# isaac-sim/IsaacGymEnvs

Measured on AMD Instinct MI355X. Metric: env-steps/sec (num_envs x control-steps/sec), random-action rollout, higher is better.
Workload: dtype f32; 1 GPU; Ant num_envs=4096 per GPU (4096 total), VecTask.step() via Python API, actions = 2*torch.rand-1 drawn before every step (README.md:48-51), seed 42+rank; 11000 untimed settle steps (about 0.5 s of back-to-back stepping at the BASELINE size) precede the 5 warm-ups; task=Ant, num_envs_per_gpu=4096, parallelism=env-shard x1, multi_wave=16, fused_sub=1, fused_post=1

## Files before the change

### isaacgymenvs_amd/csrc/core/engine_mw.hpp

```cpp
#pragma once
#include "engine.hpp"

namespace mi {

template <class M>
struct SimMW : Sim<M> {
    using B = Sim<M>;
    using typename B::Ctx;
    using typename B::BodyTmp;
    static constexpr int NB = B::NB, ND = B::ND, NV = B::NV, OFF = B::OFF, NSPH = B::NSPH, NSENS = B::NSENS, NLIM = B::NLIM,
                         NROWG = B::NROWG, NVA = B::NVA, NR = M::NROLE;

    static constexpr int role_of_body(int b) { return M::role_of_limb[M::limb_of_body[b]]; }
    static constexpr int role_of_gi(int gi) { return gi < OFF ? -1 : role_of_body(M::dof_body[gi - OFF]); }
    static constexpr bool trunk_body(int b) { return role_of_body(b) < 0; }
    static constexpr bool trunk_gi(int gi) { return role_of_gi(gi) < 0; }
    template <int R> static constexpr bool owns_body(int b) { return role_of_body(b) == R || (trunk_body(b) && R == M::TRUNK_ROLE); }
    template <int R> static constexpr bool owns_gi(int gi) { return role_of_gi(gi) == R || (trunk_gi(gi) && R == M::TRUNK_ROLE); }
    template <int R> static constexpr bool sees_gi(int gi) { return role_of_gi(gi) == R || trunk_gi(gi); }
    static constexpr int NTB = []() constexpr { int n = 0; for (int b = 0; b < NB; ++b) n += trunk_body(b) ? 1 : 0; return n; }();
    static constexpr int tslot(int b) { int n = 0; for (int k = 0; k < b; ++k) n += trunk_body(k) ? 1 : 0; return n; }
    static constexpr int NVT = []() constexpr { int n = 0; for (int i = 0; i < NV; ++i) n += trunk_gi(i) ? 1 : 0; return n; }();
    static constexpr int tidx(int gi) { int n = 0; for (int k = 0; k < gi; ++k) n += trunk_gi(k) ? 1 : 0; return n; }
    static constexpr int entry_row(int e) {
        for (int i = 0; i < NV; ++i)
            for (int j = 0; j <= i; ++j)
                if (M::midx[i][j] == e) return i;
        return 0;
    }
    static constexpr bool trunk_entry(int e) { return trunk_gi(entry_row(e)); }
    static constexpr int NTE = []() constexpr { int n = 0; for (int e = 0; e < M::NM; ++e) n += trunk_entry(e) ? 1 : 0; return n; }();
    static constexpr int teidx(int e) { int n = 0; for (int k = 0; k < e; ++k) n += trunk_entry(k) ? 1 : 0; return n; }
    static constexpr bool limb_root(int b) { return b > 0 && !trunk_body(b) && trunk_body(M::parent[b]); }
    static constexpr int NLR = []() constexpr { int n = 0; for (int b = 0; b < NB; ++b) n += limb_root(b) ? 1 : 0; return n; }();
    static constexpr int lridx(int b) { int n = 0; for (int k = 0; k < b; ++k) n += limb_root(k) ? 1 : 0; return n; }
    static constexpr int X_LR = B::ROW_SLOTS_STATIC;
    static constexpr int X_DT = X_LR + 16 * NLR;
    static constexpr int X_DY = X_DT + NR * NTE;
    static constexpr int X_DW = X_DY + NR * NVT;
    static constexpr int X_FLG = X_DW + 2 * NR * NVT;
    static constexpr int X_AT = X_FLG + 2 * NR;
    static constexpr int MW_SLOTS = X_AT + NROWG;

    static constexpr int NUNIT = NLIM + NSPH;
    template <int R> static constexpr bool own_unit(int u) {
        if (u < 0 || u >= NUNIT) return false;
        return u < NLIM ? owns_gi<R>(OFF + B::limdof(u)) : owns_body<R>(M::sph_body[u - NLIM]);
    }
    template <int R> static constexpr int next_own(int u) {
        for (int k = u + 1; k < NUNIT; ++k) if (own_unit<R>(k)) return k;
        return NUNIT;
    }
    template <int R> static constexpr int own_pos(int u) { int n = 0; for (int k = 0; k < u; ++k) n += own_unit<R>(k) ? 1 : 0; return n; }

    template <int R, int b, int XLR, int RS>
    MI_HD void trunk_down(const SimParams& P, Ctx& c, BodyTmp (&tb)[NTB], const float* Rp, const float* rp, const float* Vp,
                          const float* Ap, const RowStore<RS> rows) {
        constexpr int ts = tslot(b);
        BodyTmp& t = tb[ts];
        this->template body_down<b>(P, c, Rp, rp, Vp, Ap, t);
        sfor<NB>([&](auto C_) MI_LAMBDA {
            constexpr int ch = C_;
            if constexpr (ch > b) if constexpr (M::parent[ch] == b) {
                if constexpr (trunk_body(ch)) {
                    trunk_down<R, ch, XLR>(P, c, tb, t.Rb, t.rb, t.Vc, t.Ac, rows);
                } else if constexpr (role_of_body(ch) == R) {
                    SpI Ic;
                    float Fc[6];
                    this->template body_pass<ch>(P, c, t.Rb, t.rb, t.Vc, t.Ac, Ic, Fc);
                    constexpr int o = XLR + 16 * lridx(ch);
                    rows(o) = Ic.m;
                    sfor<3>([&](auto K) MI_LAMBDA { rows(o + 1 + K) = Ic.h[K]; });
                    sfor<6>([&](auto K) MI_LAMBDA { rows(o + 4 + K) = Ic.I[K]; rows(o + 10 + K) = Fc[K]; });
                }
            }
        });
    }

    template <int R, bool KEEP = false, int RS, class GND, class BAR>
    MI_HD void substep_role(const SimParams& P, const float* tau, const float h, const RowStore<RS> rows, const Strided lamc,
                            const Strided laml, const Strided sensor, const Strided dof_force, const GND& gnd, const float mu_env,
                            const Strided netf, const int stage, const BAR& bar) {
        static_assert(!M::FIXED, "multi-wave sub-step: free-base models");
        auto G = [&](int row, int cc) MI_LAMBDA -> float& { return rows(row * M::MAXCHAIN + cc); };
        auto Ainv = [&](int row) MI_LAMBDA -> float& { return rows(NROWG * M::MAXCHAIN + row); };
        auto vt = [&](int row) MI_LAMBDA -> float& { return rows(NROWG * M::MAXCHAIN + NROWG + row); };
        auto lam = [&](int row) MI_LAMBDA -> float& { return rows(NROWG * M::MAXCHAIN + 2 * NROWG + row); };
        const float invh = MI_RCP(h);
        float (&root)[13] = this->root;
        float (&q)[M::NDA] = this->q;
        float (&qd)[M::NDA] = this->qd;
#if defined(MI_TIMING)
        unsigned long long* const tstamp = this->tstamp;
#endif
        MI_STAMP(0);
        Ctx c;
        float (&S)[M::NDA][6] = c.S;
        float (&L)[M::NM] = c.L;
        if (stage == 0) {
            sfor<ND>([&](auto D) MI_LAMBDA {
                constexpr int d = D;
                if constexpr (M::dof_limited[d] && owns_gi<R>(OFF + d)) { constexpr int o = B::stage_slot_lim(d); rows(o) = laml(d); }
            });
            sfor<3 * NSPH>([&](auto K) MI_LAMBDA {
                if constexpr (owns_body<R>(M::sph_body[K / 3])) { constexpr int o = B::stage_slot_con(K); rows(o) = lamc(K); }
            });
        }
        BodyTmp tb[NTB];
        static_assert(!B::COMPACT && B::LAM_IN_ROWS, "substep_role: models on the static row store");
        trunk_down<R, 0, X_LR>(P, c, tb, nullptr, nullptr, nullptr, nullptr, rows);
        MI_PHASE();
        float Ldi[NVA], y[NVA], w[NVA], v[NVA];
        v[0] = root[7]; v[1] = root[8]; v[2] = root[9]; v[3] = root[10]; v[4] = root[11]; v[5] = root[12];
        sfor<ND>([&](auto D) MI_LAMBDA { v[OFF + D] = qd[D]; });
        sfor<M::NM>([&](auto E_) MI_LAMBDA { if constexpr (trunk_entry(E_)) L[E_] = 0.f; });
        sfor<NV>([&](auto I) MI_LAMBDA { if constexpr (trunk_gi(I)) y[I] = 0.f; });
        float sc_damp[M::NDA], sc_stiff[M::NDA], sc_arm[M::NDA];
        sfor<ND>([&](auto D) MI_LAMBDA { sc_damp[D] = 1.f; sc_stiff[D] = 1.f; sc_arm[D] = 1.f; });
        if constexpr (B::SCALED) {
            if (this->actor_scale.p != nullptr) {
                sfor<ND>([&](auto D) MI_LAMBDA {
                    if constexpr (sees_gi<R>(OFF + D)) {
                        sc_damp[D] = this->actor_scale(B::AS_DAMP + D); sc_stiff[D] = this->actor_scale(B::AS_STIFF + D); sc_arm[D] = this->actor_scale(B::AS_ARM + D);
                    }
                });
            }
        }
        sfor<ND>([&](auto D) MI_LAMBDA {
            constexpr int d = D, gi = OFF + d;
            if constexpr (role_of_gi(gi) == R) {
                const float K = M::dof_stiffness[d] * sc_stiff[d], Dm = M::dof_damping[d] * sc_damp[d];
                L[M::midx[gi][gi]] += M::dof_armature[d] * sc_arm[d] + h * Dm + h * h * K;
                y[gi] = tau[d] - c.bias[gi] - K * (q[d] - M::dof_springref[d]) - (Dm + h * K) * qd[d];
            }
        });
        auto factor = [&](auto K_) MI_LAMBDA {
            constexpr int k = decltype(K_)::value;
            const float dk2 = fmaxf(L[M::midx[k][k]], 1e-30f);
            const float inv = MI_RSQ(dk2);
            L[M::midx[k][k]] = dk2 * inv;
            Ldi[k] = inv;
            sfor<M::nanc[k]>([&](auto A_) MI_LAMBDA { L[M::midx[k][M::anc[k][A_]]] *= inv; });
            sfor<M::nanc[k]>([&](auto A_) MI_LAMBDA {
                constexpr int i = M::anc[k][A_];
                const float lki = L[M::midx[k][i]];
                L[M::midx[i][i]] -= lki * lki;
                sfor<M::nanc[i]>([&](auto B_) MI_LAMBDA {
                    constexpr int j = M::anc[i][B_];
                    L[M::midx[i][j]] -= lki * L[M::midx[k][j]];
                });
            });
        };
        auto whiten = [&](auto I_) MI_LAMBDA {
            constexpr int i = decltype(I_)::value;
            const float z = y[i] * Ldi[i];
            sfor<M::nanc[i]>([&](auto A_) MI_LAMBDA { y[M::anc[i][A_]] -= L[M::midx[i][M::anc[i][A_]]] * z; });
            float s = L[M::midx[i][i]] * v[i];
            sfor<M::nanc[i]>([&](auto A_) MI_LAMBDA { s += L[M::midx[i][M::anc[i][A_]]] * v[M::anc[i][A_]]; });
            w[i] = s + h * z;
        };
        sfor_rev<NV>([&](auto K_) MI_LAMBDA { if constexpr (role_of_gi(K_) == R) factor(K_); });
        MI_PHASE();
        sfor_rev<NV>([&](auto I_) MI_LAMBDA { if constexpr (role_of_gi(I_) == R) whiten(I_); });
        sfor<M::NM>([&](auto E_) MI_LAMBDA { if constexpr (trunk_entry(E_)) { constexpr int o = X_DT + R * NTE + teidx(E_); rows(o) = L[E_]; } });
        sfor<NV>([&](auto I) MI_LAMBDA { if constexpr (trunk_gi(I)) { constexpr int o = X_DY + R * NVT + tidx(I); rows(o) = y[I]; } });
// ... 86 lines not shown
                        g[kk] -= L[M::midx[i][j]] * z;
                    });
                });
                float al = P.cfm, at = 0.f;
                sfor<M::nanc[gi] + 1>([&](auto K) MI_LAMBDA {
                    constexpr int k = K, i = (k == 0) ? gi : M::anc[gi][k == 0 ? 0 : k - 1];
                    if constexpr (trunk_gi(i)) at += g[k] * g[k]; else al += g[k] * g[k];
                    G(row, k) = g[k];
                });
                Ainv(row) = al;
                rows(X_AT + row) = at;
                const float vtl = (C >= 0.f) ? -C * invh : fminf(-C * P.erp * invh, P.max_depen_vel);
                vt(row) = vtl;
                lam(row) = l0;
                act = ((l0 > 0.f) || (vtl > 0.f)) ? 1.f : act;
                wadd(std::integral_constant<int, gi>{}, g[0] * l0);
                sfor<M::nanc[gi]>([&](auto A_) MI_LAMBDA { wadd(std::integral_constant<int, M::anc[gi][A_]>{}, g[1 + A_] * l0); });
            }
        });
        MI_PHASE();
        unsigned long long sph_active = 0ull;
        sfor<NSPH>([&](auto S_) MI_LAMBDA {
            constexpr int s = S_, b = M::sph_body[s], row0 = NLIM + 3 * s;
            if constexpr (owns_body<R>(b)) {
                MI_PHASE();
                const float* cs = c.xcs[s];
                float xc[3], dist;
                float fr[3][3];
                if constexpr (GND::HEIGHTFIELD) {
                    gnd.contact(root[0] + cs[0], root[1] + cs[1], root[2] + cs[2], M::sph_rad[s], &dist, fr[0]);
                    contact_frame(fr[0], fr[1], fr[2]);
                    sfor<3>([&](auto K) MI_LAMBDA { xc[K] = cs[K] - M::sph_rad[s] * fr[0][K]; });
                } else {
                    xc[0] = cs[0]; xc[1] = cs[1]; xc[2] = cs[2] - M::sph_rad[s];
                    dist = (root[2] + xc[2]) - P.ground_z;
                }
                const bool on = dist < P.contact_offset;
                const float onf = on ? 1.f : 0.f;
                const float gap = dist - P.rest_offset;
                if (!MI_WAVE_ANY(on)) {
                    sfor<3>([&](auto K) MI_LAMBDA { lam(row0 + K) = 0.f; });
                    return;
                }
                sph_active |= 1ull << s;
                act = on ? 1.f : act;
                sfor<3>([&](auto K) MI_LAMBDA {
                    constexpr int k = K, row = row0 + k;
                    float W[6];
                    if constexpr (GND::HEIGHTFIELD) {
                        cross3(xc, fr[k], W);
                        W[3] = fr[k][0]; W[4] = fr[k][1]; W[5] = fr[k][2];
                    } else {
                        constexpr int ax = (k == 0) ? 2 : (k == 1 ? 0 : 1);
                        sfor<6>([&](auto I_) MI_LAMBDA { W[I_] = 0.f; });
                        W[3 + ax] = 1.f;
                        if constexpr (ax == 0) { W[1] = xc[2]; W[2] = -xc[1]; }
                        else if constexpr (ax == 1) { W[0] = -xc[2]; W[2] = xc[0]; }
                        else { W[0] = xc[1]; W[1] = -xc[0]; }
                    }
                    float g[M::MAXCHAIN];
                    sfor<M::chain_len[b]>([&](auto C) MI_LAMBDA {
                        constexpr int gi = M::chain[b][C];
                        if constexpr (gi >= OFF) g[C] = dot6(S[gi - OFF], W);
                        else if constexpr (gi < 3) g[C] = W[3 + gi];
                        else g[C] = W[gi - 3];
                    });
                    chain_solve(std::integral_constant<int, b>{}, g);
                    float al = P.cfm, at = 0.f;
                    sfor<M::chain_len[b]>([&](auto C) MI_LAMBDA {
                        if constexpr (trunk_gi(M::chain[b][C])) at += g[C] * g[C]; else al += g[C] * g[C];
                        G(row, C) = g[C];
                    });
                    Ainv(row) = on ? al : __builtin_inff();
                    rows(X_AT + row) = at;
                    const float vtn = (gap >= 0.f) ? -gap * invh : fminf(-gap * P.erp * invh, P.max_depen_vel);
                    if constexpr (GND::HEIGHTFIELD) vt(row) = (k == 0) ? vtn : fr[0][k - 1];
                    else vt(row) = (k == 0) ? vtn : 0.f;
                    const float l0 = lam(row) * P.warm * onf;
                    lam(row) = l0;
                    sfor<M::chain_len[b]>([&](auto C) MI_LAMBDA { wadd(std::integral_constant<int, M::chain[b][C]>{}, g[C] * l0); });
                });
            }
        });
        sfor<NVT>([&](auto I) MI_LAMBDA { rows(X_DW + R * NVT + I) = dw[I]; });
        rows(X_FLG + R) = act;
        MI_STAMP(3);
        bar();
        MI_STAMP(4);
        sfor<NV>([&](auto I) MI_LAMBDA {
            constexpr int i = I;
            if constexpr (trunk_gi(i)) { sfor<NR>([&](auto R_) MI_LAMBDA { constexpr int o = X_DW + R_ * NVT + tidx(i); w[i] += rows(o); }); }
        });
        {
            struct UBuf { float g[3][M::MAXCHAIN]; float al[3], at[3], vt, lam[3]; };
            UBuf ub[2];
            float wtl[NVT];
            for (int it = 0; it < P.iters; ++it) {
                int zero;
                MI_OPAQUE_ZERO(zero);
                const RowStore<RS> rit = rows.shifted(zero);
                const int par = it & 1;
                const RowStore<RS> xout = rows.shifted((X_DW + (par ^ 1) * NR * NVT) * RowStore<RS>::stride);
                const RowStore<RS> fin = rows.shifted((X_FLG + par * NR) * RowStore<RS>::stride), fout = rows.shifted((X_FLG + (par ^ 1) * NR) * RowStore<RS>::stride);
                float nact = 0.f;
                sfor<NR>([&](auto R_) MI_LAMBDA { nact += fin(R_); });
                const float om = (nact > 1.5f) ? 0.5f * (nact + 1.f) : 1.f;
                const float iom = 1.f / om;
                sfor<NV>([&](auto I) MI_LAMBDA { if constexpr (trunk_gi(I)) { constexpr int ti = tidx(I); wtl[ti] = w[I]; } });
                auto wget = [&](auto GI) MI_LAMBDA -> float {
                    constexpr int gi = decltype(GI)::value;
                    if constexpr (trunk_gi(gi)) { constexpr int ti = tidx(gi); return wtl[ti]; } else return w[gi];
                };
                auto wupd = [&](auto GI, const float val) MI_LAMBDA {
                    constexpr int gi = decltype(GI)::value;
                    if constexpr (trunk_gi(gi)) { constexpr int ti = tidx(gi); wtl[ti] += om * val; } else w[gi] += val;
                };
                float actn = 0.f;
                auto load_unit = [&](auto U_, UBuf& Bf) MI_LAMBDA {
                    constexpr int u = decltype(U_)::value;
                    if constexpr (u < NLIM) {
                        constexpr int d = B::limdof(u), gi = OFF + d, row = u;
                        sfor<M::nanc[gi] + 1>([&](auto K) MI_LAMBDA { Bf.g[0][K] = rit(row * M::MAXCHAIN + K); });
                        Bf.al[0] = rit(NROWG * M::MAXCHAIN + row);
                        Bf.at[0] = rit(X_AT + row);
                        Bf.vt = rit(NROWG * M::MAXCHAIN + NROWG + row);
                        Bf.lam[0] = rit(NROWG * M::MAXCHAIN + 2 * NROWG + row);
                    } else if constexpr (u < NUNIT) {
                        constexpr int s = u - NLIM, b = M::sph_body[s], row0 = NLIM + 3 * s;
                        sfor<3>([&](auto K) MI_LAMBDA {
                            sfor<M::chain_len[b]>([&](auto C) MI_LAMBDA { Bf.g[K][C] = rit((row0 + K) * M::MAXCHAIN + C); });
                            Bf.al[K] = rit(NROWG * M::MAXCHAIN + row0 + K);
                            Bf.at[K] = rit(X_AT + row0 + K);
                            Bf.lam[K] = rit(NROWG * M::MAXCHAIN + 2 * NROWG + row0 + K);
                        });
                        Bf.vt = rit(NROWG * M::MAXCHAIN + NROWG + row0);
                    }
                };
                auto unit_on = [&](auto U_) MI_LAMBDA -> bool {
                    constexpr int u = decltype(U_)::value;
                    if constexpr (u < NLIM) return true;
                    else if constexpr (u < NUNIT) return (sph_active >> (u - NLIM) & 1ull) != 0ull;
                    else return false;
                };
                constexpr int U0 = next_own<R>(-1);
                if constexpr (U0 < NUNIT) load_unit(std::integral_constant<int, U0>{}, ub[0]);
                sfor<NUNIT>([&](auto U_) MI_LAMBDA {
                    constexpr int u = U_;
                    if constexpr (own_unit<R>(u)) {
                        constexpr int pos = own_pos<R>(u), un = next_own<R>(u);
                        UBuf& Bf = ub[pos & 1];
                        if (unit_on(std::integral_constant<int, un>{}))
                            load_unit(std::integral_constant<int, un>{}, ub[(pos + 1) & 1]);
                        MI_PHASE();
                        if (!unit_on(std::integral_constant<int, u>{})) return;
                        if constexpr (u < NLIM) {
                            constexpr int d = B::limdof(u), gi = OFF + d, row = u;
                            float vn = Bf.g[0][0] * wget(std::integral_constant<int, gi>{});
                            sfor<M::nanc[gi]>([&](auto A_) MI_LAMBDA { vn += Bf.g[0][1 + A_] * wget(std::integral_constant<int, M::anc[gi][A_]>{}); });
                            const float lo = Bf.lam[0];
                            const float nl = fmaxf(lo - (vn - Bf.vt) * MI_RCP(Bf.al[0] + om * Bf.at[0]), 0.f);
                            const float dl = nl - lo;
                            lam(row) = nl;
                            actn = (nl > 0.f) ? 1.f : actn;
                            wupd(std::integral_constant<int, gi>{}, Bf.g[0][0] * dl);
                            sfor<M::nanc[gi]>([&](auto A_) MI_LAMBDA { wupd(std::integral_constant<int, M::anc[gi][A_]>{}, Bf.g[0][1 + A_] * dl); });
                        } else {
                            constexpr int s = u - NLIM, b = M::sph_body[s], row0 = NLIM + 3 * s;
                            const float mu = 0.5f * ((mu_env >= 0.f ? mu_env : M::sph_mu[s]) + P.plane_mu);
                            float ainv[3];
                            sfor<3>([&](auto K) MI_LAMBDA { ainv[K] = MI_RCP(Bf.al[K] + om * Bf.at[K]); });
                            float ln;
                            {
                                float vn = 0.f;
                                sfor<M::chain_len[b]>([&](auto C) MI_LAMBDA { vn += Bf.g[0][C] * wget(std::integral_constant<int, M::chain[b][C]>{}); });
                                const float lo = Bf.lam[0];
                                ln = fmaxf(lo - (vn - Bf.vt) * ainv[0], 0.f);
                                const float dl = ln - lo;
                                lam(row0) = ln;
                                actn = (ln > 0.f) ? 1.f : actn;
                                sfor<M::chain_len[b]>([&](auto C) MI_LAMBDA { wupd(std::integral_constant<int, M::chain[b][C]>{}, Bf.g[0][C] * dl); });
                            }
                            float lt[2], vtg[2];
                            sfor<2>([&](auto K) MI_LAMBDA {
                                float vn = 0.f;
                                sfor<M::chain_len[b]>([&](auto C) MI_LAMBDA { vn += Bf.g[1 + K][C] * wget(std::integral_constant<int, M::chain[b][C]>{}); });
                                vtg[K] = vn;
                                lt[K] = Bf.lam[1 + K] - vn * ainv[1 + K];
                            });
                            friction_disc(lt, Bf.lam[1], Bf.lam[2], vtg[0], vtg[1], ainv[1], ainv[2], mu * ln);
                            sfor<2>([&](auto K) MI_LAMBDA {
                                constexpr int row = row0 + 1 + K;
                                const float nl = lt[K], dl = nl - Bf.lam[1 + K];
                                lam(row) = nl;
                                sfor<M::chain_len[b]>([&](auto C) MI_LAMBDA { wupd(std::integral_constant<int, M::chain[b][C]>{}, Bf.g[1 + K][C] * dl); });
                            });
                        }
                    }
                });
                sfor<NV>([&](auto I) MI_LAMBDA { if constexpr (trunk_gi(I)) { constexpr int ti = tidx(I); xout(R * NVT + ti) = (wtl[ti] - w[I]) * iom; } });
                fout(R) = actn;
                bar();
                sfor<NV>([&](auto I) MI_LAMBDA {
                    constexpr int i = I;
                    if constexpr (trunk_gi(i)) { sfor<NR>([&](auto R_) MI_LAMBDA { constexpr int o = R_ * NVT + tidx(i); w[i] += xout(o); }); }
                });
            }
        }
        MI_STAMP(5);
        sfor<NV>([&](auto I_) MI_LAMBDA {
            constexpr int i = I_;
            if constexpr (sees_gi<R>(i)) {
                float s = w[i];
                sfor<M::nanc[i]>([&](auto A_) MI_LAMBDA { s -= L[M::midx[i][M::anc[i][A_]]] * v[M::anc[i][A_]]; });
                v[i] = s * Ldi[i];
            }
        });
        MI_PHASE();
        sfor<ND>([&](auto D) MI_LAMBDA {
            constexpr int d = D;
            if constexpr (owns_gi<R>(OFF + d)) {
                float ll = 0.f;
                if constexpr (M::dof_limited[d]) {
                    constexpr int row = B::limrow(d);
                    const float dl = q[d] - this->template limit_lower<d>(), du = this->template limit_upper<d>() - q[d];
                    ll = (dl < du) ? lam(row) : -lam(row);
                    if constexpr (KEEP) lam(row) = ll;
                }
                laml(d) = ll;
                dof_force(d) = tau[d] - M::dof_stiffness[d] * sc_stiff[d] * (q[d] - M::dof_springref[d]) - M::dof_damping[d] * sc_damp[d] * v[OFF + d] + ll * invh;
            }
        });
        float sens[6 * M::NSENSA];
        sfor<6 * NSENS>([&](auto K) MI_LAMBDA { sens[K] = 0.f; });
        float nf[GND::NETF ? NB : 1][3];
        if constexpr (GND::NETF) sfor<NB>([&](auto B_) MI_LAMBDA { nf[B_][0] = nf[B_][1] = nf[B_][2] = 0.f; });
        sfor<NSPH>([&](auto S_) MI_LAMBDA {
            constexpr int s = S_, b = M::sph_body[s], row0 = NLIM + 3 * s;
            if constexpr (owns_body<R>(b)) {
                if (!(sph_active >> s & 1ull)) {
                    lamc(3 * s) = 0.f; lamc(3 * s + 1) = 0.f; lamc(3 * s + 2) = 0.f;
                    return;
                }
                const float ln = lam(row0), l1 = lam(row0 + 1), l2 = lam(row0 + 2);
                lamc(3 * s) = ln; lamc(3 * s + 1) = l1; lamc(3 * s + 2) = l2;
                float f[3], xc[3];
                if constexpr (GND::HEIGHTFIELD) {
                    float n[3], t1[3], t2[3];
                    n[0] = vt(row0 + 1); n[1] = vt(row0 + 2);
                    n[2] = MI_SQRT(fmaxf(1.f - n[0] * n[0] - n[1] * n[1], 0.f));
                    contact_frame(n, t1, t2);
                    sfor<3>([&](auto K) MI_LAMBDA {
                        f[K] = (n[K] * ln + t1[K] * l1 + t2[K] * l2) * invh;
                        xc[K] = c.xcs[s][K] - M::sph_rad[s] * n[K];
                        nf[b][K] += f[K];
                    });
                } else {
                    f[0] = l1 * invh; f[1] = l2 * invh; f[2] = ln * invh;
                    xc[0] = c.xcs[s][0]; xc[1] = c.xcs[s][1]; xc[2] = c.xcs[s][2] - M::sph_rad[s];
                    if constexpr (GND::NETF) sfor<3>([&](auto K) MI_LAMBDA { nf[b][K] += f[K]; });
                }
                if constexpr (B::sensor_of(b) >= 0) {
                    constexpr int k = B::sensor_of(b);
                    const float arm[3] = {xc[0] - c.rs[k][0], xc[1] - c.rs[k][1], xc[2] - c.rs[k][2]};
                    float tq[3], fl[3], tl[3];
                    cross3(arm, f, tq);
                    matTvec3(c.Rs[k], f, fl); matTvec3(c.Rs[k], tq, tl);
                    sfor<3>([&](auto C) MI_LAMBDA { sens[6 * k + C] += fl[C]; sens[6 * k + 3 + C] += tl[C]; });
                }
            }
        });
        if constexpr (GND::NETF) sfor<NB>([&](auto B_) MI_LAMBDA {
            if constexpr (owns_body<R>(B_)) sfor<3>([&](auto K) MI_LAMBDA { netf(3 * B_ + K) = nf[B_][K]; });
        });
        sfor<NSENS>([&](auto K_) MI_LAMBDA {
            if constexpr (owns_body<R>(M::sens_body[K_])) sfor<6>([&](auto C) MI_LAMBDA { sensor(6 * K_ + C) = sens[6 * K_ + C]; });
        });
        MI_PHASE();
        sfor<ND>([&](auto D) MI_LAMBDA {
            if constexpr (owns_gi<R>(OFF + D)) { qd[D] = v[OFF + D]; q[D] += h * qd[D]; }
        });
        if constexpr (R == M::TRUNK_ROLE) {
#if !defined(MI_NO_VEL_CLAMP)
            {
                const float w2 = v[3] * v[3] + v[4] * v[4] + v[5] * v[5], l2 = v[0] * v[0] + v[1] * v[1] + v[2] * v[2];
                const float sw = (w2 > kMaxAngularVelocity * kMaxAngularVelocity) ? kMaxAngularVelocity * MI_RSQ(w2) : 1.f;
                const float sl = (l2 > kMaxLinearVelocity * kMaxLinearVelocity) ? kMaxLinearVelocity * MI_RSQ(l2) : 1.f;
                v[0] *= sl; v[1] *= sl; v[2] *= sl; v[3] *= sw; v[4] *= sw; v[5] *= sw;
            }
#endif
            sfor<3>([&](auto K) MI_LAMBDA { root[7 + K] = v[K]; root[10 + K] = v[3 + K]; root[K] += h * v[K]; });
            const float om[3] = {v[3], v[4], v[5]};
            const float an = MI_SQRT(dot3(om, om)), th = an * h;
            float dq[4];
            {
                float sn, cs;
                sincosf(0.5f * th, &sn, &cs);
                const bool big = th > 1e-12f;
                const float k = big ? sn * MI_RCP(fmaxf(an, 1e-30f)) : 0.5f * h;
                dq[0] = om[0] * k; dq[1] = om[1] * k; dq[2] = om[2] * k; dq[3] = big ? cs : 1.f;
            }
            float* Q = root + 3;
            const float x = dq[3] * Q[0] + dq[0] * Q[3] + dq[1] * Q[2] - dq[2] * Q[1];
            const float yy = dq[3] * Q[1] - dq[0] * Q[2] + dq[1] * Q[3] + dq[2] * Q[0];
            const float z = dq[3] * Q[2] + dq[0] * Q[1] - dq[1] * Q[0] + dq[2] * Q[3];
            const float ww = dq[3] * Q[3] - dq[0] * Q[0] - dq[1] * Q[1] - dq[2] * Q[2];
            const float n = MI_RSQ(x * x + yy * yy + z * z + ww * ww);
            Q[0] = x * n; Q[1] = yy * n; Q[2] = z * n; Q[3] = ww * n;
        }
        MI_STAMP(6);
    }
};

}
```

### isaacgymenvs_amd/csrc/mw_kernels.hpp

```cpp
#pragma once
#include "step_kernels.hpp"
#include "core/engine_mw.hpp"
#include "tasks/anymal_step.hpp"

namespace mi {

#if defined(MI_TIMING)
__device__ unsigned long long* g_mi_tstamp_mw = nullptr;
#endif
struct DevBarrier {
    __device__ __forceinline__ void operator()() const { __syncthreads(); }
};
template <class M, int E>
constexpr size_t mw_lds_bytes() { return (size_t)SimMW<M>::MW_SLOTS * E * sizeof(float); }
template <class M, class GND, int E, int R>
__device__ __forceinline__ void mw_role(const View& v, const SimParams& P, const ActParams& ap, const float* __restrict__ actions_in,
                                        const int src, const GND& gnd, float* lds_rows, const int e, const int lane, float* post_x = nullptr) {
    using S = SimMW<M>;
    constexpr int ND = M::ND;
    const int N = v.N;
    S sim;
    load_sim(sim, v, e);
    load_actor_scales(sim, v, e);
    float tau[M::NDA];
// ... 18 lines not shown
                    t = fminf(fmaxf(u, -ap.torque_limit), ap.torque_limit);
                }
            }
            tau[k] = t;
            if constexpr (mine) v.tau[k * N + e] = t;
        });
    } else {
        sfor<ND>([&](auto K) MI_LAMBDA { tau[K] = v.tau[K * N + e]; });
    }
    {
        typedef const __attribute__((address_space(1))) void* gptr_t;
        typedef __attribute__((address_space(3))) void* lptr_t;
        float* slot0 = lds_rows;
        sfor<ND>([&](auto D) MI_LAMBDA {
            constexpr int d = D;
            if constexpr (M::dof_limited[d] && S::template owns_gi<R>(M::OFF + d)) {
                constexpr int o = Sim<M>::stage_slot_lim(d) * E;
                __builtin_amdgcn_global_load_lds((gptr_t)(v.laml + (size_t)d * N + e), (lptr_t)(slot0 + o), 4, 0, 0);
            }
        });
        sfor<3 * M::NSPH>([&](auto K) MI_LAMBDA {
            if constexpr (S::template owns_body<R>(M::sph_body[K / 3])) {
                constexpr int o = Sim<M>::stage_slot_con(K) * E;
                __builtin_amdgcn_global_load_lds((gptr_t)(v.lamc + (size_t)K * N + e), (lptr_t)(slot0 + o), 4, 0, 0);
            }
        });
    }
    const float h = P.dt / (float)P.substeps;
    const Strided lamc{v.lamc + e, N}, laml{v.laml + e, N}, sensor{v.sensor + e, N}, dof_force{v.dof_force + e, N};
    const Strided netf{GND::NETF ? v.netf + e : nullptr, N};
    const float mu_env = (GND::HEIGHTFIELD || v.friction != nullptr) ? v.friction[e] : -1.f;
    sim.template substep_role<R>(P, tau, h, RowStore<E>{lds_rows + lane}, lamc, laml, sensor, dof_force, gnd, mu_env, netf, true, DevBarrier{});
    sfor<ND>([&](auto K) MI_LAMBDA {
        if constexpr (S::template owns_gi<R>(M::OFF + K)) {
            v.dof[K * N + e] = sim.q[K];
            v.dof[(ND + K) * N + e] = sim.qd[K];
        }
    });
    if constexpr (R == M::TRUNK_ROLE) sfor<13>([&](auto K) MI_LAMBDA { v.root[K * N + e] = sim.root[K]; });
    if (post_x != nullptr) {
        sfor<ND>([&](auto K) MI_LAMBDA {
            if constexpr (S::template owns_gi<R>(M::OFF + K)) { post_x[(13 + K) * E] = sim.q[K]; post_x[(13 + ND + K) * E] = sim.qd[K]; }
        });
        if constexpr (R == M::TRUNK_ROLE) sfor<13>([&](auto K) MI_LAMBDA { post_x[K * E] = sim.root[K]; });
    }
}
template <class M, class GND, int E>
__global__ __launch_bounds__(64 * M::NROLE) void substep_mw_kernel(View v, SimParams P, ActParams ap, const float* __restrict__ actions_in,
                                                                   int src, GND gnd) {
    extern __shared__ float lds_rows[];
    static_assert(M::NROLE == 4, "four roles, one per SIMD of a CU");
    const int lane = threadIdx.x;
    if (lane >= E) return;
    const int e = xcd_env_base<E>(blockIdx.x) + lane;
    if (e >= v.N) return;
    const int role = __builtin_amdgcn_readfirstlane(threadIdx.y);
    switch (role) {
        case 0: mw_role<M, GND, E, 0>(v, P, ap, actions_in, src, gnd, lds_rows, e, lane); break;
        case 1: mw_role<M, GND, E, 1>(v, P, ap, actions_in, src, gnd, lds_rows, e, lane); break;
        case 2: mw_role<M, GND, E, 2>(v, P, ap, actions_in, src, gnd, lds_rows, e, lane); break;
        default: mw_role<M, GND, E, 3>(v, P, ap, actions_in, src, gnd, lds_rows, e, lane); break;
    }
}

template <class GND>
struct MwFusedArgs {
    View v;
    SimParams P;
    ActParams ap;
    const float* actions_in;
    int first, rest, n_sub, tail;
    GND gnd;
    int cmdnorm = 0, cmdnorm_allow_knee = 0;
    float cmdnorm_max_len = 0.f;
};
template <class M, int E>
constexpr size_t mw_fused_lds_bytes() { return (size_t)(SimMW<M>::MW_SLOTS + 13) * E * sizeof(float); }
template <class GND>
struct MwFusedPostArgs {
    MwFusedArgs<GND> f;
    LocoParams tp;
};
template <class S, class M, bool HUM, int E, int R, bool BAR_FIRST = false>
__device__ __forceinline__ void loco_post_role(const View& v, const LocoParams& tp, S& sim, const float* act, const int e, float* xpost) {
    using T = Loco<M::ND, 6 * M::NSENS, HUM>;
    constexpr int ND = M::ND, NOBS = T::NOBS;
    const int N = v.N;
    if constexpr (BAR_FIRST) __syncthreads();
    const uint32_t genv = (uint32_t)(v.env_offset + e);
    const bool do_reset = v.reset[e] != 0;
    int ep = v.episode[e];
    float* ob = v.obs + (size_t)e * NOBS;
    float* oc = v.obs_out + ((size_t)v.ring * N + e) * NOBS;
    const float c = v.clip_obs;
    auto put = [&](const int k, const float x) MI_LAMBDA { ob[k] = x; oc[k] = fminf(fmaxf(x, -c), c); };
    sfor<ND>([&](auto D) MI_LAMBDA {
        constexpr int d = D;
        if constexpr (S::template owns_gi<R>(M::OFF + d)) {
            if (do_reset) {
                T::reset_dof(tp, v.seed, genv, (uint32_t)ep, d, tp.initial_dof_pos[d], tp.dof_lower[d], tp.dof_upper[d], &sim.q[d], &sim.qd[d]);
                v.laml[d * N + e] = 0.f;
            }
            v.dof[d * N + e] = sim.q[d];
            v.dof[(ND + d) * N + e] = sim.qd[d];
            float ps, vs, fs;
            T::obs_dof(tp, sim.q[d], sim.qd[d], HUM ? v.dof_force[d * N + e] : 0.f, tp.dof_lower[d], tp.dof_upper[d], &ps, &vs, &fs);
            const float a_d = (act != nullptr) ? act[d] : v.actions[d * N + e];
            put(T::COL_POS + d, ps);
            put(T::COL_VEL + d, vs);
            if constexpr (HUM) put(T::COL_FORCE + d, fs);
            put(T::COL_ACT + d, a_d);
            typename T::DofSums one;
            T::reward_dof(tp, a_d, ps, vs, tp.gear[d], one);
            xpost[(3 * d + 0) * E] = one.actions; xpost[(3 * d + 1) * E] = one.electricity; xpost[(3 * d + 2) * E] = one.at_limit;
        }
    });
    sfor<M::NSENS>([&](auto K_) MI_LAMBDA {
        constexpr int k = K_;
        if constexpr (S::template owns_body<R>(M::sens_body[k]))
            sfor<6>([&](auto J) MI_LAMBDA { put(T::COL_SENS + 6 * k + J, v.sensor[(6 * k + J) * N + e] * tp.contact_force_scale); });
    });
    if (do_reset) sfor<3 * M::NSPH>([&](auto K) MI_LAMBDA { if constexpr (S::template owns_body<R>(M::sph_body[K / 3])) v.lamc[K * N + e] = 0.f; });
    if constexpr (R != M::TRUNK_ROLE) { __syncthreads(); return; }
    long long progress = v.progress[e] + 1;
    float potentials = v.potentials[e], prev_potentials;
    if (do_reset) {
        float init_root[13];
        sfor<13>([&](auto K) MI_LAMBDA { init_root[K] = v.init_root[K * N + e]; sim.root[K] = init_root[K]; });
        const float pp = T::reset_potential(tp, init_root);
        potentials = pp;
        ep += 1;
        progress = 0;
        if constexpr (M::NPG > 0) { if (v.lamp) sfor<3 * M::NPG>([&](auto K) MI_LAMBDA { v.lamp[K * N + e] = 0.f; }); }
    }
    sfor<13>([&](auto K) MI_LAMBDA { v.root[K * N + e] = sim.root[K]; });
    float up_vec[3], heading_vec[3], o12[12];
    T::obs_root(tp, sim.root, tp.targets, potentials, tp.inv_start_rot, tp.basis_vec0, tp.basis_vec1, o12, &potentials, &prev_potentials, up_vec, heading_vec);
    sfor<12>([&](auto K) MI_LAMBDA { put(K, o12[K]); });
    __syncthreads();
    typename T::DofSums part[4];
    sfor<ND>([&](auto D) MI_LAMBDA {
        constexpr int d = D;
        part[d & 3].actions += xpost[(3 * d + 0) * E]; part[d & 3].electricity += xpost[(3 * d + 1) * E]; part[d & 3].at_limit += xpost[(3 * d + 2) * E];
    });
    typename T::DofSums sm;
    sm.actions = (part[0].actions + part[1].actions) + (part[2].actions + part[3].actions);
    sm.electricity = (part[0].electricity + part[1].electricity) + (part[2].electricity + part[3].electricity);
    sm.at_limit = (part[0].at_limit + part[1].at_limit) + (part[2].at_limit + part[3].at_limit);
    float rew;
    long long reset;
    T::reward_total(tp, o12[0], o12[10], o12[11], sm, 0LL, progress, potentials, prev_potentials, &rew, &reset);
    episode_stats<E, true>(v, e, true, rew, reset, progress);
    v.randomize[e] += 1;
    v.episode[e] = ep;
    v.potentials[e] = potentials;
    v.prev_potentials[e] = prev_potentials;
    sfor<3>([&](auto K) MI_LAMBDA { v.up_vec[K * N + e] = up_vec[K]; v.heading_vec[K * N + e] = heading_vec[K]; });
    v.rew[e] = rew;
    v.reset[e] = reset;
    v.progress[e] = progress;
    v.timeout[e] = (unsigned char)(((float)progress >= tp.max_episode_length - 1.f) && (reset != 0));
}

template <class M, class GND, int E, int R, bool POST = false, bool HUM = false>
__device__ __forceinline__ void mw_role_fused(const MwFusedArgs<GND>& a, float* lds_rows, const int e, const int lane, const LocoParams* tp = nullptr) {
    using S = SimMW<M>;
    constexpr int ND = M::ND;
    const View& v = a.v;
    const ActParams& ap = a.ap;
    const int N = v.N;
    S sim;
#if defined(MI_TIMING)
    unsigned long long* const tstamp = (lane == 0 && g_mi_tstamp_mw != nullptr) ? g_mi_tstamp_mw + ((size_t)blockIdx.x * 4 + R) * 32 : nullptr;
    MI_STAMP(30);
#endif
    load_sim(sim, v, e);
    load_actor_scales(sim, v, e);
    {
        typedef const __attribute__((address_space(1))) void* gptr_t;
        typedef __attribute__((address_space(3))) void* lptr_t;
        float* slot0 = lds_rows;
        sfor<ND>([&](auto D) MI_LAMBDA {
            constexpr int d = D;
            if constexpr (M::dof_limited[d] && S::template owns_gi<R>(M::OFF + d)) {
                constexpr int o = Sim<M>::stage_slot_lim(d) * E;
                __builtin_amdgcn_global_load_lds((gptr_t)(v.laml + (size_t)d * N + e), (lptr_t)(slot0 + o), 4, 0, 0);
            }
        });
        sfor<3 * M::NSPH>([&](auto K) MI_LAMBDA {
            if constexpr (S::template owns_body<R>(M::sph_body[K / 3])) {
                constexpr int o = Sim<M>::stage_slot_con(K) * E;
                __builtin_amdgcn_global_load_lds((gptr_t)(v.lamc + (size_t)K * N + e), (lptr_t)(slot0 + o), 4, 0, 0);
            }
        });
    }
    const float h = a.P.dt / (float)a.P.substeps;
    const Strided lamc{v.lamc + e, N}, laml{v.laml + e, N}, sensor{v.sensor + e, N}, dof_force{v.dof_force + e, N};
    const Strided netf{GND::NETF ? v.netf + e : nullptr, N};
    const float mu_env = (GND::HEIGHTFIELD || v.friction != nullptr) ? v.friction[e] : -1.f;
    float* xroot = lds_rows + (size_t)S::MW_SLOTS * E + lane;
    float tau[M::NDA], act[M::NDA];
    sfor<ND>([&](auto K) MI_LAMBDA { tau[K] = 0.f; act[K] = 0.f; });
    for (int i = 0; i < a.n_sub; ++i) {
        const int src = (i >= a.n_sub - a.tail) ? (i == 0 ? (int)ACT_STORED_TAU : -1) : (i == 0 ? a.first : a.rest);
        if (src == ACT_STORED_TAU) {
            if (i == 0) sfor<ND>([&](auto K) MI_LAMBDA { tau[K] = v.tau[K * N + e]; });
        } else if (src > 0) {
            sfor<ND>([&](auto K) MI_LAMBDA {
                constexpr int k = K;
                constexpr bool mine = S::template owns_gi<R>(M::OFF + k);
                float t = 0.f;
                if (k < ap.nact) {
                    float x;
                    if (src == ACT_FROM_ACTIONS) {
                        x = a.actions_in[(size_t)e * ap.nact + k];
                        x = fminf(fmaxf(x, -ap.clip), ap.clip);
                        if constexpr (mine) v.actions[k * N + e] = x;
                        act[k] = x;
                    } else if (i == 0) {
                        x = v.actions[k * N + e];
                        act[k] = x;
                    } else {
                        x = act[k];
                    }
                    if (ap.mode == 0) {
                        t = x * ap.gear[k] * ap.scale;
                    } else {
                        float qk = sim.q[k], qdk = sim.qd[k];
                        if constexpr (GND::HEIGHTFIELD) {
                            if (i == 0 && v.dof_api != nullptr) { qk = v.dof_api[k * N + e]; qdk = v.dof_api[(ND + k) * N + e]; }
                        }
                        const float u = ap.kp * (ap.scale * x + ap.gear[k] - qk) - ap.kd * qdk;
                        t = fminf(fmaxf(u, -ap.torque_limit), ap.torque_limit);
                    }
                }
                tau[k] = t;
                if constexpr (mine) v.tau[k * N + e] = t;
            });
        }
#if defined(MI_TIMING)
        sim.tstamp = (tstamp != nullptr && i < 3) ? tstamp + 8 * i : nullptr;
#endif
        sim.template substep_role<R, true>(a.P, tau, h, RowStore<E>{lds_rows + lane}, lamc, laml, sensor, dof_force, a.gnd, mu_env, netf,
                                           i == 0 ? 1 : 2, DevBarrier{});
        if constexpr (GND::HEIGHTFIELD) {
            if (i == a.n_sub - a.tail - 1 && v.dof_api != nullptr)
                sfor<ND>([&](auto K) MI_LAMBDA {
                    if constexpr (S::template owns_gi<R>(M::OFF + K)) { v.dof_api[K * N + e] = sim.q[K]; v.dof_api[(ND + K) * N + e] = sim.qd[K]; }
                });
        }
        if (i + 1 < a.n_sub) {
            if constexpr (R == M::TRUNK_ROLE) sfor<13>([&](auto K) MI_LAMBDA { xroot[K * E] = sim.root[K]; });
            __syncthreads();
            if constexpr (R != M::TRUNK_ROLE) sfor<13>([&](auto K) MI_LAMBDA { sim.root[K] = xroot[K * E]; });
        }
    }
    if constexpr (GND::HEIGHTFIELD && !POST) {
        if (a.cmdnorm != 0) {
            __syncthreads();
            if constexpr (R == M::TRUNK_ROLE) {
                bool rs = anymal_netf_norm(v, e, 0) > 1.f;
                if (a.cmdnorm_allow_knee == 0)
                    for (int k = 0; k < 4; ++k) rs = rs || (anymal_netf_norm(v, e, anymal_knee_body(k)) > 1.f);
                if (v.progress[e] + 1 >= (long long)a.cmdnorm_max_len - 1) rs = true;
                float acc = 0.f;
                if (rs) { const float cx = v.commands[e], cy = v.commands[N + e]; acc = cx * cx + cy * cy; }
                acc = wave_sum_live<E>(acc);
                if ((threadIdx.x & 63) == 0 && acc > 0.f) atomicAdd(v.ep_stats + 15, acc);
            }
        }
    }
    if constexpr (POST) {
        static_assert(3 * M::ND <= 16 * S::NLR, "the reward terms fit the (by now dead) tree-pass exchange area");
        loco_post_role<S, M, HUM, E, R>(v, *tp, sim, act, e, lds_rows + (size_t)S::X_LR * E + lane);
        MI_STAMP(31);
        return;
    }
    sfor<ND>([&](auto K) MI_LAMBDA {
        if constexpr (S::template owns_gi<R>(M::OFF + K)) {
            v.dof[K * N + e] = sim.q[K];
            v.dof[(ND + K) * N + e] = sim.qd[K];
        }
    });
    if constexpr (R == M::TRUNK_ROLE) sfor<13>([&](auto K) MI_LAMBDA { v.root[K * N + e] = sim.root[K]; });
}
template <class M, class GND, int E, bool HUM>
__global__ __launch_bounds__(64 * M::NROLE, E == 8 ? 2 : 1) void substep_mw_fused_post_kernel(MwFusedPostArgs<GND> args_by_value) {
    extern __shared__ float lds_rows[];
    static_assert(M::NROLE == 4, "four roles, one per SIMD of a CU");
#if defined(__HIP_DEVICE_COMPILE__)
    (void)args_by_value;
    const MwFusedPostArgs<GND>& a = *reinterpret_cast<const MwFusedPostArgs<GND>*>(__builtin_amdgcn_kernarg_segment_ptr());
    const int lane = threadIdx.x;
    if (lane >= E) return;
    const int e = xcd_env_base<E>(blockIdx.x) + lane;
    if (e >= a.f.v.N) return;
    const int role = __builtin_amdgcn_readfirstlane(threadIdx.y);
    switch (role) {
        case 0: mw_role_fused<M, GND, E, 0, true, HUM>(a.f, lds_rows, e, lane, &a.tp); break;
        case 1: mw_role_fused<M, GND, E, 1, true, HUM>(a.f, lds_rows, e, lane, &a.tp); break;
        case 2: mw_role_fused<M, GND, E, 2, true, HUM>(a.f, lds_rows, e, lane, &a.tp); break;
        default: mw_role_fused<M, GND, E, 3, true, HUM>(a.f, lds_rows, e, lane, &a.tp); break;
    }
#endif
}
template <class M, class GND, int E>
__global__ __launch_bounds__(64 * M::NROLE) void substep_mw_fused_kernel(MwFusedArgs<GND> args_by_value) {
    extern __shared__ float lds_rows[];
    static_assert(M::NROLE == 4, "four roles, one per SIMD of a CU");
#if defined(__HIP_DEVICE_COMPILE__)
    (void)args_by_value;
    const MwFusedArgs<GND>& a = *reinterpret_cast<const MwFusedArgs<GND>*>(__builtin_amdgcn_kernarg_segment_ptr());
    const int lane = threadIdx.x;
    if (lane >= E) return;
    const int e = xcd_env_base<E>(blockIdx.x) + lane;
    if (e >= a.v.N) return;
    const int role = __builtin_amdgcn_readfirstlane(threadIdx.y);
    switch (role) {
        case 0: mw_role_fused<M, GND, E, 0>(a, lds_rows, e, lane); break;
        case 1: mw_role_fused<M, GND, E, 1>(a, lds_rows, e, lane); break;
        case 2: mw_role_fused<M, GND, E, 2>(a, lds_rows, e, lane); break;
        default: mw_role_fused<M, GND, E, 3>(a, lds_rows, e, lane); break;
    }
#endif
}

template <class M, class GND>
hipError_t launch_substeps_mw(const View& v, const SimParams& P, const ActParams& ap, const float* actions, int n_sub, int first, int rest,
                              hipStream_t s, const GND& gnd, int tail, const MwCmdNormTail* cn) {
    const dim3 block(64, M::NROLE);
    if (v.fused_sub != 0 && n_sub > 1) {
        static unsigned long long fconf16 = 0ull, fconf32 = 0ull;
        constexpr size_t flds16 = mw_fused_lds_bytes<M, 16>(), flds32 = mw_fused_lds_bytes<M, 32>();
        MwFusedArgs<GND> fa{v, P, ap, actions, first, rest, n_sub, tail, gnd};
        if (cn != nullptr) { fa.cmdnorm = 1; fa.cmdnorm_allow_knee = cn->allow_knee_contacts; fa.cmdnorm_max_len = cn->max_episode_length; }
        if (MI_MW_HAS16 && v.mw == 16) {
            auto kern = substep_mw_fused_kernel<M, GND, MI_MW_HAS16 ? 16 : 32>;
            if (hipError_t e = ensure_dynamic_lds((const void*)kern, flds16, &fconf16); e != hipSuccess) return e;
            hipLaunchKernelGGL(kern, dim3(xcd_grid<16>(v.N)), block, flds16, s, fa);
        } else {
            auto kern = substep_mw_fused_kernel<M, GND, 32>;
            if (hipError_t e = ensure_dynamic_lds((const void*)kern, flds32, &fconf32); e != hipSuccess) return e;
            hipLaunchKernelGGL(kern, dim3(xcd_grid<32>(v.N)), block, flds32, s, fa);
        }
        return hipGetLastError();
    }
    static unsigned long long conf16 = 0ull, conf32 = 0ull;
    constexpr size_t lds16 = mw_lds_bytes<M, 16>(), lds32 = mw_lds_bytes<M, 32>();
    auto src_of = [&](int i) { return i >= n_sub - tail ? (int)ACT_STORED_TAU : (i == 0 ? first : rest); };
    if (MI_MW_HAS16 && v.mw == 16) {
        auto kern = substep_mw_kernel<M, GND, MI_MW_HAS16 ? 16 : 32>;
        if (hipError_t e = ensure_dynamic_lds((const void*)kern, lds16, &conf16); e != hipSuccess) return e;
        const dim3 grid(xcd_grid<16>(v.N));
        for (int i = 0; i < n_sub; ++i) hipLaunchKernelGGL(kern, grid, block, lds16, s, v, P, ap, actions, src_of(i), gnd);
    } else {
        auto kern = substep_mw_kernel<M, GND, 32>;
        if (hipError_t e = ensure_dynamic_lds((const void*)kern, lds32, &conf32); e != hipSuccess) return e;
// ... 93 lines not shown
```

Measured before the change: 95.24 million env-steps/s.

## Prefetch solver rows across barriers and skip redundant per-substep global outputs

Moves the first constraint-unit prefetch ahead of the barrier and re-prefetches the next iteration's first unit before the end-of-iteration barrier, so the LDS loads overlap the synchronisation. The trunk weight is computed once per iteration right after the barrier, not at the start of each loop. Global writes of tau, limit lambdas, dof forces, sensors and net forces now happen only on the last sub-step for flat ground. Sensor values are also passed to the fused post-processing in registers, and actions are loaded before the sub-step loop. This trims redundant global memory traffic and barrier stalls, at the cost of more live registers and some more complex control flow.

```diff
diff --git a/isaacgymenvs_amd/csrc/core/engine_mw.hpp b/isaacgymenvs_amd/csrc/core/engine_mw.hpp
--- a/isaacgymenvs_amd/csrc/core/engine_mw.hpp
+++ b/isaacgymenvs_amd/csrc/core/engine_mw.hpp
@@ -80,7 +80,7 @@
     template <int R, bool KEEP = false, int RS, class GND, class BAR>
     MI_HD void substep_role(const SimParams& P, const float* tau, const float h, const RowStore<RS> rows, const Strided lamc,
                             const Strided laml, const Strided sensor, const Strided dof_force, const GND& gnd, const float mu_env,
-                            const Strided netf, const int stage, const BAR& bar) {
+                            const Strided netf, const int stage, const BAR& bar, const bool outs = true, float* sens_out = nullptr) {
         static_assert(!M::FIXED, "multi-wave sub-step: free-base models");
         auto G = [&](int row, int cc) MI_LAMBDA -> float& { return rows(row * M::MAXCHAIN + cc); };
         auto Ainv = [&](int row) MI_LAMBDA -> float& { return rows(NROWG * M::MAXCHAIN + row); };
@@ -333,18 +333,58 @@
                 });
             }
         });
+        struct UBuf { float g[3][M::MAXCHAIN]; float al[3], at[3], vt, lam[3]; };
+        UBuf ub[2];
+        auto load_unit = [&](auto U_, UBuf& Bf, const RowStore<RS>& rit) MI_LAMBDA {
+            constexpr int u = decltype(U_)::value;
+            if constexpr (u < NLIM) {
+                constexpr int d = B::limdof(u), gi = OFF + d, row = u;
+                sfor<M::nanc[gi] + 1>([&](auto K) MI_LAMBDA { Bf.g[0][K] = rit(row * M::MAXCHAIN + K); });
+                Bf.al[0] = rit(NROWG * M::MAXCHAIN + row);
+                Bf.at[0] = rit(X_AT + row);
+                Bf.vt = rit(NROWG * M::MAXCHAIN + NROWG + row);
+                Bf.lam[0] = rit(NROWG * M::MAXCHAIN + 2 * NROWG + row);
+            } else if constexpr (u < NUNIT) {
+                constexpr int s = u - NLIM, b = M::sph_body[s], row0 = NLIM + 3 * s;
+                sfor<3>([&](auto K) MI_LAMBDA {
+                    sfor<M::chain_len[b]>([&](auto C) MI_LAMBDA { Bf.g[K][C] = rit((row0 + K) * M::MAXCHAIN + C); });
+                    Bf.al[K] = rit(NROWG * M::MAXCHAIN + row0 + K);
+                    Bf.at[K] = rit(X_AT + row0 + K);
+                    Bf.lam[K] = rit(NROWG * M::MAXCHAIN + 2 * NROWG + row0 + K);
+                });
+                Bf.vt = rit(NROWG * M::MAXCHAIN + NROWG + row0);
+            }
+        };
+        auto unit_on = [&](auto U_) MI_LAMBDA -> bool {
+            constexpr int u = decltype(U_)::value;
+            if constexpr (u < NLIM) return true;
+            else if constexpr (u < NUNIT) return (sph_active >> (u - NLIM) & 1ull) != 0ull;
+            else return false;
+        };
+        constexpr int U0 = next_own<R>(-1);
+        {
+            int zero;
+            MI_OPAQUE_ZERO(zero);
+            if (unit_on(std::integral_constant<int, U0>{})) load_unit(std::integral_constant<int, U0>{}, ub[0], rows.shifted(zero));
+        }
         sfor<NVT>([&](auto I) MI_LAMBDA { rows(X_DW + R * NVT + I) = dw[I]; });
         rows(X_FLG + R) = act;
         MI_STAMP(3);
         bar();
         MI_STAMP(4);
+        float om, iom;
+        auto trunk_weight = [&](const RowStore<RS>& flg) MI_LAMBDA {
+            float nact = 0.f;
+            sfor<NR>([&](auto R_) MI_LAMBDA { nact += flg(R_); });
+            om = (nact > 1.5f) ? 0.5f * (nact + 1.f) : 1.f;
+            iom = 1.f / om;
+        };
+        trunk_weight(rows.shifted(X_FLG * RowStore<RS>::stride));
         sfor<NV>([&](auto I) MI_LAMBDA {
             constexpr int i = I;
             if constexpr (trunk_gi(i)) { sfor<NR>([&](auto R_) MI_LAMBDA { constexpr int o = X_DW + R_ * NVT + tidx(i); w[i] += rows(o); }); }
         });
         {
-            struct UBuf { float g[3][M::MAXCHAIN]; float al[3], at[3], vt, lam[3]; };
-            UBuf ub[2];
             float wtl[NVT];
             for (int it = 0; it < P.iters; ++it) {
                 int zero;
@@ -352,11 +392,7 @@
                 const RowStore<RS> rit = rows.shifted(zero);
                 const int par = it & 1;
                 const RowStore<RS> xout = rows.shifted((X_DW + (par ^ 1) * NR * NVT) * RowStore<RS>::stride);
-                const RowStore<RS> fin = rows.shifted((X_FLG + par * NR) * RowStore<RS>::stride), fout = rows.shifted((X_FLG + (par ^ 1) * NR) * RowStore<RS>::stride);
-                float nact = 0.f;
-                sfor<NR>([&](auto R_) MI_LAMBDA { nact += fin(R_); });
-                const float om = (nact > 1.5f) ? 0.5f * (nact + 1.f) : 1.f;
-                const float iom = 1.f / om;
+                const RowStore<RS> fout = rows.shifted((X_FLG + (par ^ 1) * NR) * RowStore<RS>::stride);
                 sfor<NV>([&](auto I) MI_LAMBDA { if constexpr (trunk_gi(I)) { constexpr int ti = tidx(I); wtl[ti] = w[I]; } });
                 auto wget = [&](auto GI) MI_LAMBDA -> float {
                     constexpr int gi = decltype(GI)::value;
@@ -367,41 +403,13 @@
                     if constexpr (trunk_gi(gi)) { constexpr int ti = tidx(gi); wtl[ti] += om * val; } else w[gi] += val;
                 };
                 float actn = 0.f;
-                auto load_unit = [&](auto U_, UBuf& Bf) MI_LAMBDA {
-                    constexpr int u = decltype(U_)::value;
-                    if constexpr (u < NLIM) {
-                        constexpr int d = B::limdof(u), gi = OFF + d, row = u;
-                        sfor<M::nanc[gi] + 1>([&](auto K) MI_LAMBDA { Bf.g[0][K] = rit(row * M::MAXCHAIN + K); });
-                        Bf.al[0] = rit(NROWG * M::MAXCHAIN + row);
-                        Bf.at[0] = rit(X_AT + row);
-                        Bf.vt = rit(NROWG * M::MAXCHAIN + NROWG + row);
-                        Bf.lam[0] = rit(NROWG * M::MAXCHAIN + 2 * NROWG + row);
-                    } else if constexpr (u < NUNIT) {
-                        constexpr int s = u - NLIM, b = M::sph_body[s], row0 = NLIM + 3 * s;
-                        sfor<3>([&](auto K) MI_LAMBDA {
-                            sfor<M::chain_len[b]>([&](auto C) MI_LAMBDA { Bf.g[K][C] = rit((row0 + K) * M::MAXCHAIN + C); });
-                            Bf.al[K] = rit(NROWG * M::MAXCHAIN + row0 + K);
-                            Bf.at[K] = rit(X_AT + row0 + K);
-                            Bf.lam[K] = rit(NROWG * M::MAXCHAIN + 2 * NROWG + row0 + K);
-                        });
-                        Bf.vt = rit(NROWG * M::MAXCHAIN + NROWG + row0);
-                    }
-                };
-                auto unit_on = [&](auto U_) MI_LAMBDA -> bool {
-                    constexpr int u = decltype(U_)::value;
-                    if constexpr (u < NLIM) return true;
-                    else if constexpr (u < NUNIT) return (sph_active >> (u - NLIM) & 1ull) != 0ull;
-                    else return false;
-                };
-                constexpr int U0 = next_own<R>(-1);
-                if constexpr (U0 < NUNIT) load_unit(std::integral_constant<int, U0>{}, ub[0]);
                 sfor<NUNIT>([&](auto U_) MI_LAMBDA {
                     constexpr int u = U_;
                     if constexpr (own_unit<R>(u)) {
                         constexpr int pos = own_pos<R>(u), un = next_own<R>(u);
                         UBuf& Bf = ub[pos & 1];
                         if (unit_on(std::integral_constant<int, un>{}))
-                            load_unit(std::integral_constant<int, un>{}, ub[(pos + 1) & 1]);
+                            load_unit(std::integral_constant<int, un>{}, ub[(pos + 1) & 1], rit);
                         MI_PHASE();
                         if (!unit_on(std::integral_constant<int, u>{})) return;
                         if constexpr (u < NLIM) {
@@ -448,9 +456,11 @@
                         }
                     }
                 });
+                if (unit_on(std::integral_constant<int, U0>{})) load_unit(std::integral_constant<int, U0>{}, ub[0], rit);
                 sfor<NV>([&](auto I) MI_LAMBDA { if constexpr (trunk_gi(I)) { constexpr int ti = tidx(I); xout(R * NVT + ti) = (wtl[ti] - w[I]) * iom; } });
                 fout(R) = actn;
                 bar();
+                trunk_weight(fout);
                 sfor<NV>([&](auto I) MI_LAMBDA {
                     constexpr int i = I;
                     if constexpr (trunk_gi(i)) { sfor<NR>([&](auto R_) MI_LAMBDA { constexpr int o = R_ * NVT + tidx(i); w[i] += xout(o); }); }
@@ -477,10 +487,13 @@
                     ll = (dl < du) ? lam(row) : -lam(row);
                     if constexpr (KEEP) lam(row) = ll;
                 }
-                laml(d) = ll;
-                dof_force(d) = tau[d] - M::dof_stiffness[d] * sc_stiff[d] * (q[d] - M::dof_springref[d]) - M::dof_damping[d] * sc_damp[d] * v[OFF + d] + ll * invh;
-            }
-        });
+                if (outs) {
+                    laml(d) = ll;
+                    dof_force(d) = tau[d] - M::dof_stiffness[d] * sc_stiff[d] * (q[d] - M::dof_springref[d]) - M::dof_damping[d] * sc_damp[d] * v[OFF + d] + ll * invh;
+                }
+            }
+        });
+        if (outs) {
         float sens[6 * M::NSENSA];
         sfor<6 * NSENS>([&](auto K) MI_LAMBDA { sens[K] = 0.f; });
         float nf[GND::NETF ? NB : 1][3];
@@ -524,8 +537,12 @@
             if constexpr (owns_body<R>(B_)) sfor<3>([&](auto K) MI_LAMBDA { netf(3 * B_ + K) = nf[B_][K]; });
         });
         sfor<NSENS>([&](auto K_) MI_LAMBDA {
-            if constexpr (owns_body<R>(M::sens_body[K_])) sfor<6>([&](auto C) MI_LAMBDA { sensor(6 * K_ + C) = sens[6 * K_ + C]; });
-        });
+            if constexpr (owns_body<R>(M::sens_body[K_])) sfor<6>([&](auto C) MI_LAMBDA {
+                sensor(6 * K_ + C) = sens[6 * K_ + C];
+                if (sens_out != nullptr) sens_out[6 * K_ + C] = sens[6 * K_ + C];
+            });
+        });
+        }
         MI_PHASE();
         sfor<ND>([&](auto D) MI_LAMBDA {
             if constexpr (owns_gi<R>(OFF + D)) { qd[D] = v[OFF + D]; q[D] += h * qd[D]; }
diff --git a/isaacgymenvs_amd/csrc/mw_kernels.hpp b/isaacgymenvs_amd/csrc/mw_kernels.hpp
--- a/isaacgymenvs_amd/csrc/mw_kernels.hpp
+++ b/isaacgymenvs_amd/csrc/mw_kernels.hpp
@@ -124,7 +124,8 @@
     LocoParams tp;
 };
 template <class S, class M, bool HUM, int E, int R, bool BAR_FIRST = false>
-__device__ __forceinline__ void loco_post_role(const View& v, const LocoParams& tp, S& sim, const float* act, const int e, float* xpost) {
+__device__ __forceinline__ void loco_post_role(const View& v, const LocoParams& tp, S& sim, const float* act, const int e, float* xpost,
+                                               const float* sens = nullptr) {
     using T = Loco<M::ND, 6 * M::NSENS, HUM>;
     constexpr int ND = M::ND, NOBS = T::NOBS;
     const int N = v.N;
@@ -160,7 +161,10 @@
     sfor<M::NSENS>([&](auto K_) MI_LAMBDA {
         constexpr int k = K_;
         if constexpr (S::template owns_body<R>(M::sens_body[k]))
-            sfor<6>([&](auto J) MI_LAMBDA { put(T::COL_SENS + 6 * k + J, v.sensor[(6 * k + J) * N + e] * tp.contact_force_scale); });
+            sfor<6>([&](auto J) MI_LAMBDA {
+                const float sv = (sens != nullptr) ? sens[6 * k + J] : v.sensor[(6 * k + J) * N + e];
+                put(T::COL_SENS + 6 * k + J, sv * tp.contact_force_scale);
+            });
     });
     if (do_reset) sfor<3 * M::NSPH>([&](auto K) MI_LAMBDA { if constexpr (S::template owns_body<R>(M::sph_body[K / 3])) v.lamc[K * N + e] = 0.f; });
     if constexpr (R != M::TRUNK_ROLE) { __syncthreads(); return; }
@@ -216,6 +220,15 @@
     unsigned long long* const tstamp = (lane == 0 && g_mi_tstamp_mw != nullptr) ? g_mi_tstamp_mw + ((size_t)blockIdx.x * 4 + R) * 32 : nullptr;
     MI_STAMP(30);
 #endif
+    float tau[M::NDA], act[M::NDA];
+    sfor<ND>([&](auto K) MI_LAMBDA { tau[K] = 0.f; act[K] = 0.f; });
+    if ((a.first == ACT_FROM_ACTIONS || a.rest == ACT_FROM_ACTIONS) && ap.nact > 0) {
+        const float* arow = a.actions_in + (size_t)e * ap.nact;
+        sfor<ND>([&](auto K) MI_LAMBDA {
+            constexpr int k = K;
+            if constexpr (S::template sees_gi<R>(M::OFF + k)) act[k] = arow[k < ap.nact ? k : ap.nact - 1];
+        });
+    }
     load_sim(sim, v, e);
     load_actor_scales(sim, v, e);
     {
@@ -241,8 +254,10 @@
     const Strided netf{GND::NETF ? v.netf + e : nullptr, N};
     const float mu_env = (GND::HEIGHTFIELD || v.friction != nullptr) ? v.friction[e] : -1.f;
     float* xroot = lds_rows + (size_t)S::MW_SLOTS * E + lane;
-    float tau[M::NDA], act[M::NDA];
-    sfor<ND>([&](auto K) MI_LAMBDA { tau[K] = 0.f; act[K] = 0.f; });
+    float sens[POST ? 6 * M::NSENSA : 1];
+    if constexpr (POST) sfor<6 * M::NSENS>([&](auto K) MI_LAMBDA { sens[K] = 0.f; });
+    const int last_eval = (a.rest == ACT_STORED_TAU) ? 0 : a.n_sub - a.tail - 1;
+    constexpr bool ALL_OUTS = GND::HEIGHTFIELD;
     for (int i = 0; i < a.n_sub; ++i) {
         const int src = (i >= a.n_sub - a.tail) ? (i == 0 ? (int)ACT_STORED_TAU : -1) : (i == 0 ? a.first : a.rest);
         if (src == ACT_STORED_TAU) {
@@ -255,8 +270,7 @@
                 if (k < ap.nact) {
                     float x;
                     if (src == ACT_FROM_ACTIONS) {
-                        x = a.actions_in[(size_t)e * ap.nact + k];
-                        x = fminf(fmaxf(x, -ap.clip), ap.clip);
+                        x = fminf(fmaxf(act[k], -ap.clip), ap.clip);
                         if constexpr (mine) v.actions[k * N + e] = x;
                         act[k] = x;
                     } else if (i == 0) {
@@ -277,14 +291,14 @@
                     }
                 }
                 tau[k] = t;
-                if constexpr (mine) v.tau[k * N + e] = t;
+                if constexpr (mine) { if (ALL_OUTS || i == last_eval) v.tau[k * N + e] = t; }
             });
         }
 #if defined(MI_TIMING)
         sim.tstamp = (tstamp != nullptr && i < 3) ? tstamp + 8 * i : nullptr;
 #endif
         sim.template substep_role<R, true>(a.P, tau, h, RowStore<E>{lds_rows + lane}, lamc, laml, sensor, dof_force, a.gnd, mu_env, netf,
-                                           i == 0 ? 1 : 2, DevBarrier{});
+                                           i == 0 ? 1 : 2, DevBarrier{}, ALL_OUTS || i + 1 == a.n_sub, POST ? sens : nullptr);
         if constexpr (GND::HEIGHTFIELD) {
             if (i == a.n_sub - a.tail - 1 && v.dof_api != nullptr)
                 sfor<ND>([&](auto K) MI_LAMBDA {
@@ -314,7 +328,7 @@
     }
     if constexpr (POST) {
         static_assert(3 * M::ND <= 16 * S::NLR, "the reward terms fit the (by now dead) tree-pass exchange area");
-        loco_post_role<S, M, HUM, E, R>(v, *tp, sim, act, e, lds_rows + (size_t)S::X_LR * E + lane);
+        loco_post_role<S, M, HUM, E, R>(v, *tp, sim, act, e, lds_rows + (size_t)S::X_LR * E + lane, sens);
         MI_STAMP(31);
         return;
     }
```

After: 96.12 million env-steps/s, median of 6. No clear change (+0.9%).
